# ChainSafe/co-zkvms

Measured on AMD Instinct MI355X. Metric: RISC-V cycles proved/sec (co-Jolt hot path: PST13 commit + dense GKR grand product + openings), higher is better.
Workload: dtype u32-limb BN254 Fr/Fq (254-bit Montgomery integers); 1 GPU; configs[1] restated (SURVEY 8d): 2^20-cycle trace per GPU, plain prover, 128 polys (64 Fr + 32 u16 + 16 u32 + 16 flags) PST13 batch commit, dense grand product 8 x 2^21 leaves, batch evaluate + opening reduction + PST13 open; log_n=20, polys=128, gp_batch=8, parallelism=single GPU, ranks_per_gpu=1

## Files before the change

co-zkvms_amd/csrc/capi.hip:

```cpp
#include "common.hpp"
#include "fq9.hip.hpp"
#include "prf.hip.hpp"

static __device__ __forceinline__ uint64_t splitmix_next(uint64_t& s) {
    s += 0x9E3779B97F4A7C15ull;
    uint64_t z = s;
    z = (z ^ (z >> 30)) * 0xBF58476D1CE4E5B9ull;
    z = (z ^ (z >> 27)) * 0x94D049BB133111EBull;
    return z ^ (z >> 31);
}

__global__ void k_fill_random_fr(fe* out, size_t n, uint64_t seed, int max_bits) {
    size_t i = (size_t)blockIdx.x * blockDim.x + threadIdx.x;
    if (i >= n) return;
    uint64_t s = seed + (uint64_t)i * 0xD1342543DE82EF95ull;
    fe v;
    for (;;) {
        uint64_t w0 = splitmix_next(s), w1 = splitmix_next(s), w2 = splitmix_next(s);
        uint64_t w3 = splitmix_next(s) & ((1ull << 62) - 1ull);
        v.l[0] = (uint32_t)w0; v.l[1] = (uint32_t)(w0 >> 32);
        v.l[2] = (uint32_t)w1; v.l[3] = (uint32_t)(w1 >> 32);
        v.l[4] = (uint32_t)w2; v.l[5] = (uint32_t)(w2 >> 32);
        v.l[6] = (uint32_t)w3; v.l[7] = (uint32_t)(w3 >> 32);
        if (!Fr::geq_mod(v)) break;
// ... 116 lines not shown
    {
        std::lock_guard<std::mutex> lk(g_ctx_mu);
        g_live_ctx.insert(ctx);
    }
    *out = ctx;
    return COZK_OK;
}

int cozk_ctx_destroy(cozk_ctx* ctx) {
    if (!ctx) return COZK_OK;
    {
        std::lock_guard<std::mutex> lk(g_ctx_mu);
        g_live_ctx.erase(ctx);
    }
    (void)hipSetDevice(ctx->device);
    (void)hipStreamSynchronize(ctx->stream);
    if (ctx->ring_comm) (void)cozk_ring_destroy(ctx);
    ctx->pool.destroy();
    for (auto& pr : ctx->prof_events) {
        (void)hipEventDestroy(pr.first);
        (void)hipEventDestroy(pr.second);
    }
    for (ProfSlot& sl : ctx->prof_slots) sl.reset();
    ctx->msm_ws.release();
    ctx->scratch.release();
    ctx->scratch2.release();
    if (ctx->pinned) (void)hipHostFree(ctx->pinned);
    if (ctx->round_flag) (void)hipHostFree(ctx->round_flag);
    if (ctx->finish_ticket) (void)hipFree(ctx->finish_ticket);
    if (ctx->mailbox) (void)hipHostFree(ctx->mailbox);
    if (ctx->stream2) {
        (void)hipStreamSynchronize(ctx->stream2);
        (void)hipStreamDestroy(ctx->stream2);
    }
    (void)hipStreamDestroy(ctx->stream);
    delete ctx;
    return COZK_OK;
}

int cozk_ctx_set_resident_rounds(cozk_ctx* ctx, int enable) {
    if (!ctx) return COZK_ERR_INVALID_ARG;
    ctx->resident_rounds = enable > 0 ? 1 : (enable == 0 ? 0 : -1);
    return COZK_OK;
}

const char* cozk_last_error(cozk_ctx* ctx) { return ctx ? ctx->last_error.c_str() : "null context"; }

int cozk_ctx_synchronize(cozk_ctx* ctx) {
    return cozk_guard(ctx, [&] { HIP_TRY(hipStreamSynchronize(ctx->stream)); });
}

int cozk_ctx_stream(cozk_ctx* ctx, void** out_stream) {
    if (!ctx || !out_stream) return COZK_ERR_INVALID_ARG;
    *out_stream = (void*)ctx->stream;
    return COZK_OK;
}

int cozk_vec_alloc(cozk_ctx* ctx, size_t n, int kind, cozk_vec** out) {
    return cozk_guard(ctx, [&] {
        COZK_REQUIRE(ctx && out && scalar_kind_bytes(kind), "vec_alloc: bad argument");
        size_t bytes = n * scalar_kind_bytes(kind);
        void* d = ctx_dev_alloc(ctx, bytes);
        *out = new cozk_vec{ctx, n, kind, d, bytes, true};
    });
}

// ... 233 lines not shown
```

co-zkvms_amd/csrc/common.hpp:

```cpp
#pragma once
#ifdef COZK_COUNT_COPIES
#include <hip/hip_runtime.h>
#include <map>
#include <string>
#include <cstdio>
#include <mutex>
struct CozkCopyCounter {
    std::map<std::string, unsigned long> m;
    std::mutex mu;
    ~CozkCopyCounter() {
        for (auto& kv : m) fprintf(stderr, "[copies] %8lu  %s\n", kv.second, kv.first.c_str());
    }
};
inline CozkCopyCounter& cozk_copy_counter() { static CozkCopyCounter c; return c; }
inline void cozk_count_copy(const char* what, const char* f, int l) {
    auto& c = cozk_copy_counter();
    std::lock_guard<std::mutex> g(c.mu);
    const char* b = f;
    for (const char* p = f; *p; p++) if (*p == '/') b = p + 1;
    c.m[std::string(what) + " " + b + ":" + std::to_string(l)]++;
}
#define hipMemcpyAsync(...) (cozk_count_copy("memcpy", __FILE__, __LINE__), hipMemcpyAsync(__VA_ARGS__))
#define hipStreamSynchronize(...) (cozk_count_copy("sync", __FILE__, __LINE__), hipStreamSynchronize(__VA_ARGS__))
#define hipMemsetAsync(...) (cozk_count_copy("memset", __FILE__, __LINE__), hipMemsetAsync(__VA_ARGS__))
// ... 41 lines not shown
    void reserve(size_t bytes) {
        if (bytes <= cap) return;
        if (p) HIP_TRY(hipFree(p));
        p = nullptr;
        cap = 0;
        if (hipMalloc(&p, bytes) != hipSuccess) {
            (void)hipGetLastError();
            p = nullptr;
            trim_current_pool();
            HIP_TRY(hipMalloc(&p, bytes));
        }
        cap = bytes;
    }
    void release() {
        if (p) (void)hipFree(p);
        p = nullptr;
        cap = 0;
    }
    template <class T>
    T* as() { return reinterpret_cast<T*>(p); }
};

struct MsmSortWs {
    DevBuf hist, off0, refs, offA, ptrs;
    hipEvent_t done = nullptr, consumed = nullptr;
    void release() {
        for (DevBuf* b : {&hist, &off0, &refs, &offA, &ptrs}) b->release();
        for (hipEvent_t* e : {&done, &consumed}) {
            if (*e) (void)hipEventDestroy(*e);
            *e = nullptr;
        }
    }
};
struct MsmWorkspace {
    MsmSortWs sort[2];
    DevBuf offB, offC, heavy, partA, partB, bsum, chunk, grp, out, ptrs, exc, blk, perm, offP, form, corr;
    hipEvent_t fork = nullptr;
    void* pin = nullptr;
    size_t pin_cap = 0;
    void release() {
        for (MsmSortWs& s : sort) s.release();
        for (DevBuf* b : {&offB, &offC, &heavy, &partA, &partB, &bsum, &chunk, &grp, &out, &ptrs, &exc, &blk, &perm, &offP, &form, &corr}) b->release();
        if (pin) (void)hipHostFree(pin);
        pin = nullptr;
        pin_cap = 0;
        if (fork) (void)hipEventDestroy(fork);
        fork = nullptr;
    }
};

struct DevPool {
    std::unordered_map<size_t, std::vector<void*>> parked;
    std::unordered_map<void*, size_t> live;
    size_t parked_bytes = 0;
    size_t live_bytes = 0, peak_bytes = 0;
    void count(size_t c) {
        live_bytes += c;
        if (live_bytes > peak_bytes) peak_bytes = live_bytes;
    }
    static size_t size_class(size_t bytes) {
        if (bytes <= 256) return 256;
        size_t top = (size_t)1 << (63 - __builtin_clzll((unsigned long long)bytes));
        size_t q = top >> 2;
        return (bytes + q - 1) / q * q;
    }
    void trim() {
        for (auto& kv : parked)
            for (void* p : kv.second) (void)hipFree(p);
        parked.clear();
        parked_bytes = 0;
    }
    void* alloc(size_t bytes) {
        size_t c = size_class(bytes);
        auto it = parked.find(c);
        if (it != parked.end() && !it->second.empty()) {
            void* p = it->second.back();
            it->second.pop_back();
            parked_bytes -= c;
            live[p] = c;
            count(c);
// ... 23 lines not shown
        trim();
        for (auto& kv : live) (void)hipFree(kv.first);
        live.clear();
    }
};

enum {
    COZK_PROF_EVAL_CHI = 0,
    COZK_PROF_LINCOMB,
    COZK_PROF_BIND_CUBIC,
    COZK_PROF_MSM_SCATTER,
    COZK_PROF_LAYER_OUTPUT,
    COZK_PROF_SLOTS
};
struct ProfSlot {
    std::vector<std::pair<hipEvent_t, hipEvent_t>> events;
    double ms = 0.0;
    uint64_t launches = 0, alg_bytes = 0;
    void reset() {
        for (auto& pr : events) {
            (void)hipEventDestroy(pr.first);
            (void)hipEventDestroy(pr.second);
        }
        events.clear();
        ms = 0.0;
        launches = alg_bytes = 0;
    }
};

struct cozk_ctx {
    int device = 0;
    hipStream_t stream = nullptr;
    hipStream_t stream2 = nullptr;
    DevPool pool;
    std::string last_error;
    MsmWorkspace msm_ws;
    DevBuf scratch;
    DevBuf scratch2;
    void* pinned = nullptr;
    size_t pinned_cap = 0;
    int resident_rounds = -1;
    void* mailbox = nullptr;
    uint32_t* round_flag = nullptr;
    uint32_t round_seq = 0;
    uint32_t armed_seq = 0;
    unsigned* finish_ticket = nullptr;
    bool prof_enabled = false;
    std::vector<std::pair<hipEvent_t, hipEvent_t>> prof_events;
    double prof_ms = 0.0;
    uint64_t prof_launches = 0;
    uint64_t prof_units = 0;
    uint64_t prof_alg_bytes = 0;
    ProfSlot prof_slots[COZK_PROF_SLOTS];
    void* ring_comm = nullptr;
    int ring_rank = 0, ring_n = 0;
    uint64_t ring_bytes = 0;
    cozk_sparse_stats sparse_stats{};
};

struct ProfScope {
    cozk_ctx* ctx;
    hipStream_t st;
    int slot;
    hipEvent_t e0 = nullptr, e1 = nullptr;
    ProfScope(cozk_ctx* c, int slot_, uint64_t alg_bytes, hipStream_t stream = nullptr) : ctx(c), st(stream ? stream : c->stream), slot(slot_) {
        if (!ctx->prof_enabled) return;
// ... 123 lines not shown
```

co-zkvms_amd/csrc/msm.hip:

```cpp
#include "common.hpp"
#include "fq9.hip.hpp"
#include <cstring>

static constexpr uint32_t NB = 1u << 15;
static constexpr int CH = 16;
static constexpr int TPB = 256;

template <int KIND>
struct ScalarKind;
template <>
struct ScalarKind<COZK_SCALAR_FR> {
    static constexpr int NWIN = 16;
    static __device__ __forceinline__ bool load(const void* p, size_t i, uint32_t w[8]) {
        fe s = Fr::from_mont(fe_load(reinterpret_cast<const fe*>(p) + i));
#pragma unroll
        for (int k = 0; k < 8; k++) w[k] = s.l[k];
        return false;
    }
};
template <>
struct ScalarKind<COZK_SCALAR_U8> {
    static constexpr int NWIN = 1;
    static __device__ __forceinline__ bool load(const void* p, size_t i, uint32_t w[8]) {
        w[0] = reinterpret_cast<const uint8_t*>(p)[i];
// ... 749 lines not shown
        if (m > pl.bound) pl.bound = m;
    }
    COZK_REQUIRE(pl.M < (1ull << 32), "msm: batch too large (reference count exceeds 32 bits)");
    uint32_t L0 = (uint32_t)(pl.M >> 18);
    if (L0 < 8) L0 = 8;
    if (L0 > 127) L0 = 127;
    pl.L0 = L0;
    pl.maxseg0 = pl.M / L0 + pl.nb;
    uint64_t per = 0;
    for (size_t p = 0; p < P; p++) {
        uint64_t m = ((uint64_t)ns[p] * (pl.pre ? kind_nwin(kinds[p]) : 1) + NB - 1) / NB;
        if (m > per) per = m;
    }
    uint64_t segs = (per * 5 + 4 * L0 - 1) / (4 * L0) + 1;
    pl.fold_levels = 1;
    while ((segs = (segs + 7) / 8) > 1) pl.fold_levels++;
    return pl;
}

static void msm_scan(hipStream_t st, uint32_t* bsums, uint32_t nb, bool from_offsets, const uint32_t* in, uint32_t L, uint32_t* off, uint32_t* cursor,
                     const uint32_t* perm = nullptr) {
    const uint32_t nscan_blocks = (nb + SCAN_PER_BLOCK - 1) / SCAN_PER_BLOCK;
    if (from_offsets) {
        k_scan_sums<true><<<nscan_blocks, 256, 0, st>>>(in, nb, L, bsums, perm);
        k_scan_top<<<1, 1024, 0, st>>>(bsums, nscan_blocks, off + nb);
        k_scan_final<true><<<nscan_blocks, 256, 0, st>>>(in, nb, L, bsums, off, cursor, perm);
    } else {
        k_scan_sums<false><<<nscan_blocks, 256, 0, st>>>(in, nb, L, bsums, nullptr);
        k_scan_top<<<1, 1024, 0, st>>>(bsums, nscan_blocks, off + nb);
        k_scan_final<false><<<nscan_blocks, 256, 0, st>>>(in, nb, L, bsums, off, cursor, nullptr);
    }
}

static void msm_sort(cozk_ctx* ctx, hipStream_t st, MsmSortWs& sw, const MsmSetPlan& pl, const cozk_bases* bases, const size_t* offsets,
                     const size_t* ns, const void* const* scalars, const int* kinds) {
    const uint32_t nb = pl.nb, G = pl.G;
    const size_t P = pl.P;
    sw.hist.reserve((size_t)(nb + 3) * 4);
    sw.off0.reserve((size_t)(nb + 1) * 4);
    sw.offA.reserve((size_t)(nb + 1) * 4);
    sw.refs.reserve((size_t)pl.M * 4);
    uint32_t* hist = sw.hist.as<uint32_t>();
    uint32_t* off0 = sw.off0.as<uint32_t>();
    uint32_t* refs = sw.refs.as<uint32_t>();
    const uint32_t nscan_blocks = (nb + SCAN_PER_BLOCK - 1) / SCAN_PER_BLOCK;
    sw.ptrs.reserve((size_t)nscan_blocks * 4 + P * sizeof(MsmPolyDesc) + 64);
    uint32_t* bsums = sw.ptrs.as<uint32_t>();
    MsmPolyDesc* d_descs = reinterpret_cast<MsmPolyDesc*>(((uintptr_t)(bsums + nscan_blocks) + 15) & ~(uintptr_t)15);
    HIP_TRY(hipMemsetAsync(hist, 0, (size_t)(nb + 3) * 4, st));
    uint32_t* d_stats = hist + nb + 1;
    auto fullest_bucket = [&] { k_max_u32<<<std::min<uint32_t>(cdiv(nb, 256), 1024u), 256, 0, st>>>(hist, nb, d_stats); };
    auto read_back_stats = [&] {
        k_msm_set_total<<<1, 1, 0, st>>>(off0 + nb, d_stats);
        HIP_TRY(hipMemcpyAsync(&pl.pin->fullest, d_stats, 8, hipMemcpyDeviceToHost, st));
    };
    if (pl.pre) {
        MsmPolyDesc* h_descs = pl.pin->descs;
        COZK_REQUIRE(P <= 64, "msm: too many polynomials in one launch set");
        uint32_t nd = 0;
        struct KindRun { int kind; uint32_t first, count; size_t max_n; uint32_t wgs; };
        std::vector<KindRun> runs;
        size_t max_n = 0;
        for (int kind = 0; kind <= COZK_SCALAR_I64; kind++) {
            KindRun r{kind, nd, 0, 0, 0};
            for (size_t p = 0; p < P; p++)
                if (kinds[p] == kind && ns[p]) {
                    h_descs[nd++] = MsmPolyDesc{scalars[p], (uint32_t)ns[p], (uint32_t)offsets[p], (uint32_t)p, 0};
                    if (ns[p] > r.max_n) r.max_n = ns[p];
                }
            r.count = nd - r.first;
            if (r.max_n > max_n) max_n = r.max_n;
            if (r.count) runs.push_back(r);
        }
        HIP_TRY(hipMemcpyAsync(d_descs, h_descs, nd * sizeof(MsmPolyDesc), hipMemcpyHostToDevice, st));
        static const int ltpb_env = getenv("COZK_MSM_LTPB") ? atoi(getenv("COZK_MSM_LTPB")) : 0;
        static const int wgs_env = getenv("COZK_MSM_WGS") ? atoi(getenv("COZK_MSM_WGS")) : 0;
        const int ltpb = ltpb_env ? ltpb_env : (pl.wide ? MSM_WIDE_LTPB : 256);
        const uint32_t wgs_max = (uint32_t)(wgs_env ? wgs_env : (pl.wide ? MSM_WIDE_WGS : 64));
        COZK_REQUIRE(ltpb >= 64 && ltpb <= LTPB && ltpb % 64 == 0, "COZK_MSM_LTPB out of range");
// ... 22 lines not shown
        fullest_bucket();
        msm_scan(st, bsums, nb, false, hist, 1, off0, hist);
        read_back_stats();
        for (auto& r : runs) {
            dim3 grid(r.wgs, r.count);
            uint64_t alg = 0;
            for (uint32_t q = 0; q < r.count; q++) {
                const MsmPolyDesc& d = h_descs[r.first + q];
                const uint64_t sb = scalar_kind_bytes(r.kind);
                alg += (uint64_t)d.n * (sb + 4ull * ((sb * 8 + 15) / 16));
            }
            ProfScope prof(ctx, COZK_PROF_MSM_SCATTER, alg, st);
            KIND_DISPATCH(r.kind, (k_msm_scatter_lds<K><<<grid, ltpb, 0, st>>>(d_descs + r.first, hist, refs, (uint32_t)bases->n, pl.form)));
        }
    } else {
        for (size_t p = 0; p < P; p++) {
            uint32_t* h = hist + (size_t)p * G * NB;
            if (ns[p]) KIND_DISPATCH(kinds[p], (k_msm_hist<K><<<cdiv(ns[p], TPB), TPB, 0, st>>>(scalars[p], ns[p], h, 1)));
        }
        fullest_bucket();
        msm_scan(st, bsums, nb, false, hist, 1, off0, hist);
        read_back_stats();
        for (size_t p = 0; p < P; p++) {
            uint32_t* cur = hist + (size_t)p * G * NB;
            if (ns[p])
                KIND_DISPATCH(kinds[p], (k_msm_scatter<K><<<cdiv(ns[p], TPB), TPB, 0, st>>>(scalars[p], ns[p], cur, refs, 1, (uint32_t)bases->n,
                                                                                         (uint32_t)offsets[p])));
        }
    }
    msm_scan(st, bsums, nb, true, off0, pl.L0, sw.offA.as<uint32_t>(), nullptr);
    HIP_TRY(hipGetLastError());
}

static void msm_accumulate(cozk_ctx* ctx, MsmSortWs& sw, const MsmSetPlan& pl, const cozk_bases* bases, const size_t* ns, const int* kinds,
                           g1_xyzz* dense_out) {
    MsmWorkspace& ws = ctx->msm_ws;
    hipStream_t st = ctx->stream;
    const uint32_t nb = pl.nb, L0 = pl.L0;
    const uint32_t L1 = 8;
    const uint64_t maxseg0 = pl.maxseg0;
    const uint64_t maxpart = maxseg0 > 2ull * nb ? maxseg0 : 2ull * nb;
    ws.partA.reserve((size_t)maxpart * sizeof(g1_xyzz));
    ws.partB.reserve((size_t)maxpart * sizeof(g1_xyzz));
    ws.offB.reserve((size_t)(nb + 1) * 4);
    ws.offC.reserve((size_t)(nb + 1) * 4);
    ws.heavy.reserve((size_t)(nb + 1) * 4);
    ws.ptrs.reserve((size_t)((nb + SCAN_PER_BLOCK - 1) / SCAN_PER_BLOCK) * 4 + 64);
    uint32_t* refs = sw.refs.as<uint32_t>();
    uint32_t* off0 = sw.off0.as<uint32_t>();
    uint32_t* offA = sw.offA.as<uint32_t>();
    hipEvent_t e0 = nullptr, e1 = nullptr;
    if (ctx->prof_enabled) {
        HIP_TRY(hipEventCreate(&e0));
        HIP_TRY(hipEventCreate(&e1));
        HIP_TRY(hipEventRecord(e0, st));
    }
    ws.blk.reserve((size_t)(cdiv(maxpart, TPB) + 2) * 4);
    uint32_t* blk = ws.blk.as<uint32_t>();
    if (pl.pre) {
        ws.exc.reserve((size_t)(maxseg0 + 2) * 4);
        uint32_t* exc = ws.exc.as<uint32_t>();
        HIP_TRY(hipMemsetAsync(exc, 0, 4, st));
        ws.perm.reserve((size_t)nb * 4);
        ws.offP.reserve((size_t)(nb + 1) * 4 + SEGKEYS * 4);
        uint32_t* perm = ws.perm.as<uint32_t>();
        uint32_t* offP = ws.offP.as<uint32_t>();
        uint32_t* bins = offP + nb + 1;
        HIP_TRY(hipMemsetAsync(bins, 0, SEGKEYS * 4, st));
        k_seg_hist<<<cdiv(nb, 1024), 1024, 0, st>>>(off0, offA, nb, bins);
        k_seg_bins<<<1, 1, 0, st>>>(bins);
        k_seg_perm<<<cdiv(nb, 1024), 1024, 0, st>>>(off0, offA, nb, bins, perm);
        msm_scan(st, ws.ptrs.as<uint32_t>(), nb, true, offA, 1, offP, nullptr, perm);
        const uint32_t nblk0 = cdiv(maxseg0, TPB);
        k_block_buckets<<<cdiv(nblk0 + 1, 256), 256, 0, st>>>(offP, nb, nblk0, blk);
        if (bases->has_inf)
            k_msm_accum0_f9<true><<<nblk0, TPB, 0, st>>>(bases->table, refs, off0, offA, nb, ws.partA.as<g1_xyzz>(), exc, blk, offP, perm);
        else
            k_msm_accum0_f9<false, true><<<nblk0, TPB, 0, st>>>(bases->table, refs, off0, offA, nb, ws.partA.as<g1_xyzz>(), exc, blk, offP, perm);
        k_msm_accum0_fix<<<256, TPB, 0, st>>>(bases->table, refs, off0, offA, nb, ws.partA.as<g1_xyzz>(), exc, offP, perm);
    } else {
        k_msm_accum0<<<cdiv(maxseg0, TPB), TPB, 0, st>>>(bases->table, refs, off0, offA, nb, L0, ws.partA.as<g1_xyzz>());
    }
    if (ctx->prof_enabled) {
        HIP_TRY(hipEventRecord(e1, st));
        ctx->prof_events.push_back({e0, e1});
        ctx->prof_launches += 1;
        for (size_t p = 0; p < pl.P; p++) ctx->prof_alg_bytes += (uint64_t)ns[p] * (64 + scalar_kind_bytes(kinds[p]));
    }
    uint32_t* heavy = ws.heavy.as<uint32_t>();
    HIP_TRY(hipMemsetAsync(heavy, 0, 4, st));
    uint64_t maxseg = maxseg0;
    g1_xyzz* cur_items = ws.partA.as<g1_xyzz>();
    g1_xyzz* nxt_items = ws.partB.as<g1_xyzz>();
    uint32_t* cur_off = offA;
    uint32_t* nxt_off = ws.offB.as<uint32_t>();
    uint32_t* spare_off = ws.offC.as<uint32_t>();
    for (uint32_t level = 0; level < pl.fold_levels; level++) {
        uint64_t nseg = maxseg / L1 + nb;
        msm_scan(st, ws.ptrs.as<uint32_t>(), nb, true, cur_off, L1, nxt_off, nullptr);
        const uint32_t nblkN = cdiv(nseg, TPB);
        k_block_buckets<<<cdiv(nblkN + 1, 256), 256, 0, st>>>(nxt_off, nb, nblkN, blk);
        k_msm_accumN<<<nblkN, TPB, 0, st>>>(cur_items, cur_off, nxt_off, nb, L1, nxt_items, blk);
        std::swap(cur_items, nxt_items);
        uint32_t* done = cur_off;
        cur_off = nxt_off;
        nxt_off = (done == offA) ? spare_off : done;
        maxseg = nseg;
    }
    k_msm_gather_buckets<<<cdiv(nb, TPB), TPB, 0, st>>>(cur_items, cur_off, nb, dense_out, heavy);
    k_msm_fold_heavy<<<HEAVY_GRID, TPB, 0, st>>>(cur_items, cur_off, heavy, dense_out);
    HIP_TRY(hipGetLastError());
}

static void affine_to_abi(const g1_affine& a, uint64_t xy[8], int* inf) {
    bool is_inf = G1::is_inf(a);
    for (int i = 0; i < 4; i++) {
        xy[i] = (uint64_t)a.x.l[2 * i] | ((uint64_t)a.x.l[2 * i + 1] << 32);
        xy[4 + i] = (uint64_t)a.y.l[2 * i] | ((uint64_t)a.y.l[2 * i + 1] << 32);
    }
    if (inf) *inf = is_inf ? 1 : 0;
}
static g1_affine abi_to_affine(const uint64_t xy[8], int inf) {
    g1_affine a;
    for (int i = 0; i < 4; i++) {
        a.x.l[2 * i] = (uint32_t)xy[i];
        a.x.l[2 * i + 1] = (uint32_t)(xy[i] >> 32);
        a.y.l[2 * i] = (uint32_t)xy[4 + i];
        a.y.l[2 * i + 1] = (uint32_t)(xy[4 + i] >> 32);
    }
    if (inf) {
        a.x = Fq::zero();
        a.y = Fq::zero();
    }
    return a;
}

void msm_batch(cozk_ctx* ctx, const cozk_bases* bases, const size_t* offsets, const size_t* ns, const void* const* scalars,
               const int* kinds, size_t k, uint64_t* out_xy, int* out_inf);

enum { MSM_FORM_AUTO = 0, MSM_FORM_PLAIN = 1, MSM_FORM_OFFSET = 2 };
static int msm_digit_form_mode() {
    const char* e = getenv("COZK_MSM_DIGIT_FORM");
    if (!e || !*e || !strcmp(e, "auto")) return MSM_FORM_AUTO;
    if (!strcmp(e, "plain")) return MSM_FORM_PLAIN;
    if (!strcmp(e, "offset")) return MSM_FORM_OFFSET;
    throw CozkError(COZK_ERR_INVALID_ARG, "COZK_MSM_DIGIT_FORM must be auto, plain or offset");
}

struct MsmSchedule {
    bool shape_rule = true;
    int wg_digits_log2 = MSM_WG_DIGITS_LOG2;
};
static MsmSchedule msm_schedule_env() {
    MsmSchedule s;
    if (const char* e = getenv("COZK_MSM_SHAPE_RULE")) s.shape_rule = atoi(e) != 0;
    if (const char* e = getenv("COZK_MSM_WG_DIGITS_LOG2")) {
        s.wg_digits_log2 = atoi(e);
        COZK_REQUIRE(s.wg_digits_log2 == 0 || (s.wg_digits_log2 >= 10 && s.wg_digits_log2 <= 24), "COZK_MSM_WG_DIGITS_LOG2 must be 0 or 10..24");
    }
    return s;
}

static constexpr size_t MSM_SLICE_SUMS = 32;
static cozk_bases::SliceSum msm_slice_sum(cozk_ctx* ctx, const cozk_bases* bases, size_t off, size_t n) {
    cozk_bases* b = const_cast<cozk_bases*>(bases);
    {
        std::lock_guard<std::mutex> lk(b->sums_mu);
        for (const auto& e : b->sums)
            if (e.off == off && e.n == n) return e;
    }
    void* ones = ctx_dev_alloc(ctx, n);
    uint64_t xy[8];
    int inf = 0;
    try {
        HIP_TRY(hipMemsetAsync(ones, 1, n, ctx->stream));
        const void* p = ones;
        int kind = COZK_SCALAR_U8;
        msm_batch(ctx, bases, &off, &n, &p, &kind, 1, xy, &inf);
    } catch (...) {
        ctx_dev_free(ctx, ones);
        throw;
    }
    ctx_dev_free(ctx, ones);
    const g1_affine S = abi_to_affine(xy, inf);
    cozk_bases::SliceSum e;
    e.off = off;
    e.n = n;
    const uint64_t c[3] = {0x8000ull, 0x80008000ull, 0x8000800080008000ull};
    for (int j = 0; j < 3; j++) {
        g1_xyzz acc = G1::identity();
        for (int bit = 63; bit >= 0; bit--) {
            acc = G1::dbl(acc);
            if ((c[j] >> bit) & 1ull) acc = G1::add_mixed(acc, S);
        }
        e.cS[j] = G1::to_affine(acc);
    }
    std::lock_guard<std::mutex> lk(b->sums_mu);
    for (const auto& have : b->sums)
        if (have.off == off && have.n == n) return have;
    if (b->sums.size() >= MSM_SLICE_SUMS) b->sums.erase(b->sums.begin());
    b->sums.push_back(e);
    return e;
}

void msm_batch(cozk_ctx* ctx, const cozk_bases* bases, const size_t* offsets, const size_t* ns, const void* const* scalars,
               const int* kinds, size_t k, uint64_t* out_xy, int* out_inf) {
    MsmWorkspace& ws = ctx->msm_ws;
    hipStream_t st = ctx->stream;
    const uint32_t G = bases->nwin == 16 ? 1u : 16u;
    const size_t maxP = bases->nwin == 16 ? 64 : 4;
    const size_t tail_cap = 256 / G;
    const int form_mode = msm_digit_form_mode();
    const MsmSchedule sched = msm_schedule_env();
    std::vector<uint8_t> elig(k, 0);
    std::vector<g1_affine> corr_h;
    bool any_elig = false;
    if (G == 1 && form_mode != MSM_FORM_PLAIN) {
        for (size_t p = 0; p < k; p++) {
            const int slot = kind_offset_slot(kinds[p]);
            if (slot < 0 || ns[p] == 0) continue;
            COZK_REQUIRE(offsets[p] + ns[p] <= bases->n, "msm: base slice out of range");
            if (!any_elig) corr_h.assign(k, g1_affine{Fq::zero(), Fq::zero()});
            any_elig = true;
            elig[p] = 1;
            if (p > 0 && elig[p - 1] && kinds[p - 1] == kinds[p] && offsets[p - 1] == offsets[p] && ns[p - 1] == ns[p]) corr_h[p] = corr_h[p - 1];
            else corr_h[p] = msm_slice_sum(ctx, bases, offsets[p], ns[p]).cS[slot];
        }
    }
    ws.out.reserve(k * sizeof(g1_affine));
    g1_affine* d_out = ws.out.as<g1_affine>();
    const size_t pin_need = k * (sizeof(MsmSetPin) + sizeof(g1_affine));
    if (pin_need > ws.pin_cap) {
        if (ws.pin) (void)hipHostFree(ws.pin);
        ws.pin = nullptr;
        ws.pin_cap = 0;
        HIP_TRY(hipHostMalloc(&ws.pin, pin_need, hipHostMallocDefault));
        ws.pin_cap = pin_need;
    }
    MsmSetPin* pins = reinterpret_cast<MsmSetPin*>(ws.pin);
// ... 32 lines not shown
                if (set_refs_cap < (1ull << 28)) set_refs_cap = 1ull << 28;
                if (set_refs_cap > (1ull << 30)) set_refs_cap = 1ull << 30;
            }
        }
        {
            size_t s = 0;
            while (s < kt) {
                size_t P = 0;
                uint64_t M = 0;
                while (s + P < kt && P < maxP) {
                    uint64_t m = (uint64_t)ns[t0 + s + P] * kind_nwin(kinds[t0 + s + P]);
                    if (P > 0 && M + m > set_refs_cap) break;
                    M += m;
                    P++;
                }
                sets.push_back({s, P});
                s += P;
            }
        }
        if (sets.size() > 2) {
            size_t best = 0;
            uint64_t best_m = ~0ull;
            for (size_t i = 0; i < sets.size(); i++) {
                uint64_t m = 0;
                for (size_t p = 0; p < sets[i].P; p++) m += (uint64_t)ns[t0 + sets[i].s + p] * kind_nwin(kinds[t0 + sets[i].s + p]);
                if (m < best_m) {
                    best_m = m;
                    best = i;
                }
            }
            std::rotate(sets.begin(), sets.begin() + best, sets.begin() + best + 1);
        }
        static const bool pipeline = getenv("COZK_MSM_SERIAL") == nullptr;
        hipStream_t side = st;
        if (pipeline && sets.size() > 1) {
            if (!ctx->stream2) {
                static const bool prio = getenv("COZK_MSM_NO_PRIORITY") == nullptr;
                int lo = 0, hi = 0;
                HIP_TRY(hipDeviceGetStreamPriorityRange(&lo, &hi));
                if (prio) HIP_TRY(hipStreamCreateWithPriority(&ctx->stream2, hipStreamNonBlocking, hi));
                else HIP_TRY(hipStreamCreateWithFlags(&ctx->stream2, hipStreamNonBlocking));
            }
            side = ctx->stream2;
        }
        for (int b = 0; b < 2; b++) {
            if (!ws.sort[b].done) HIP_TRY(hipEventCreateWithFlags(&ws.sort[b].done, hipEventDisableTiming));
            if (!ws.sort[b].consumed) HIP_TRY(hipEventCreateWithFlags(&ws.sort[b].consumed, hipEventDisableTiming));
        }
        if (side != st) {
            if (!ws.fork) HIP_TRY(hipEventCreateWithFlags(&ws.fork, hipEventDisableTiming));
            HIP_TRY(hipEventRecord(ws.fork, st));
            HIP_TRY(hipStreamWaitEvent(side, ws.fork, 0));
        }
        std::vector<MsmSetPlan> plans(sets.size());
        auto launch_sort = [&](size_t i) {
            const SetRange& r = sets[i];
            plans[i] = msm_plan(bases, offsets + t0 + r.s, ns + t0 + r.s, kinds + t0 + r.s, r.P);
            if (plans[i].M == 0) return;
            MsmSetPlan& pl = plans[i];
            pl.pin = pins + pins_used++;
            pl.pin->fullest = 0;
            pl.pin->total = 0;
            pin_bound.push_back(pl.bound);
            pl.form = any_elig ? d_form + t0 + r.s : nullptr;
            pl.counts = any_elig ? d_counts + 2 * (t0 + r.s) : nullptr;
            for (size_t p = 0; p < r.P; p++)
                if (elig[t0 + r.s + p]) pl.elig |= 1ull << p;
            pl.force_offset = form_mode == MSM_FORM_OFFSET;
            const uint64_t pred_refs = i > 0 && side != st ? plans[i - 1].M : 0;
            pl.wide = sched.shape_rule ? msm_sort_wide(pred_refs, pl.M) : (i == 0 && t0 == 0) || side == st;
            pl.wg_digits_log2 = sched.wg_digits_log2;
            pl.index = (uint32_t)i;
            MsmSortWs& sw = ws.sort[i & 1];
            if (i >= 2 && side != st) HIP_TRY(hipStreamWaitEvent(side, sw.consumed, 0));
            msm_sort(ctx, side, sw, plans[i], bases, offsets + t0 + r.s, ns + t0 + r.s, scalars + t0 + r.s, kinds + t0 + r.s);
            if (side != st) HIP_TRY(hipEventRecord(sw.done, side));
        };
        if (!sets.empty()) launch_sort(0);
        for (size_t i = 0; i < sets.size(); i++) {
            if (side != st && i + 1 < sets.size()) launch_sort(i + 1);
            const SetRange& r = sets[i];
            g1_xyzz* out_i = dense + (size_t)r.s * G * NB;
            if (plans[i].M != 0) {
                MsmSortWs& sw = ws.sort[i & 1];
                if (side != st) HIP_TRY(hipStreamWaitEvent(st, sw.done, 0));
                msm_accumulate(ctx, sw, plans[i], bases, ns + t0 + r.s, kinds + t0 + r.s, out_i);
                if (side != st) HIP_TRY(hipEventRecord(sw.consumed, st));
            } else {
                HIP_TRY(hipMemsetAsync(out_i, 0, (size_t)plans[i].nb * sizeof(g1_xyzz), st));
            }
            if (side == st && i + 1 < sets.size()) launch_sort(i + 1);
        }
        k_msm_reduce_chunks<<<cdiv((uint64_t)ngroups * (NB / CH), TPB), TPB, 0, st>>>(dense, ngroups, ws.chunk.as<g1_xyzz>());
        k_msm_reduce_groups<<<ngroups, TPB, 0, st>>>(ws.chunk.as<g1_xyzz>(), ws.grp.as<g1_xyzz>());
        k_msm_finalize<<<cdiv(kt, 64), 64, 0, st>>>(ws.grp.as<g1_xyzz>(), G, (uint32_t)kt, d_out + t0, d_form ? d_form + t0 : nullptr,
                                                   d_corr ? d_corr + t0 : nullptr);
        HIP_TRY(hipGetLastError());
    }
    g1_affine* h = reinterpret_cast<g1_affine*>(ctx_pinned(ctx, k * sizeof(g1_affine)));
    HIP_TRY(hipMemcpyAsync(h, d_out, k * sizeof(g1_affine), hipMemcpyDeviceToHost, st));
    HIP_TRY(hipStreamSynchronize(st));
    for (size_t i = 0; i < pins_used; i++) {
        COZK_REQUIRE(pins[i].fullest <= pin_bound[i], "msm: histogram larger than the reference count");
        if (ctx->prof_enabled) ctx->prof_units += pins[i].total;
    }
    for (size_t i = 0; i < k; i++) affine_to_abi(h[i], out_xy + 8 * i, out_inf ? out_inf + i : nullptr);
}

extern "C" {

int cozk_bases_upload(cozk_ctx* ctx, const uint64_t* xy, const uint8_t* infinity, size_t n, int precompute,
                      cozk_bases** out) {
    return cozk_guard(ctx, [&] {
        COZK_REQUIRE(ctx && xy && out && n > 0, "bases_upload: bad argument");
        cozk_bases* b = new cozk_bases{ctx, n, precompute ? 16 : 1, nullptr};
        try {
            HIP_TRY(hipMalloc((void**)&b->table, (size_t)b->nwin * n * sizeof(g1_affine)));
            std::vector<g1_affine> h(n);
            for (size_t i = 0; i < n; i++) h[i] = abi_to_affine(xy + 8 * i, infinity ? infinity[i] : 0);
            HIP_TRY(hipMemcpyAsync(b->table, h.data(), n * sizeof(g1_affine), hipMemcpyHostToDevice, ctx->stream));
            HIP_TRY(hipStreamSynchronize(ctx->stream));
            build_window_table(ctx, b);
            HIP_TRY(hipStreamSynchronize(ctx->stream));
        } catch (...) {
            if (b->table) (void)hipFree(b->table);
            delete b;
            throw;
// ... 216 lines not shown
```

Before: 9.248 million cycles/s.

## Run MSM bucket folds on a third stream with per-set reduction tails

Splits MSM accumulation into a gather phase on the main stream and a fold phase on a new third stream. Fold workspaces are double-buffered and all buffers are reserved up front, draining the streams if a buffer must grow. The per-set reduce kernels are also issued right after each set's fold instead of once at the end. The aim is to overlap the fold and reduce tail of one set with the sort and gather of the next set. The cost is an extra device-to-device copy of offA per set, more events and cross-stream waits, and higher memory use from duplicated fold buffers.

```diff
diff --git a/co-zkvms_amd/csrc/capi.hip b/co-zkvms_amd/csrc/capi.hip
--- a/co-zkvms_amd/csrc/capi.hip
+++ b/co-zkvms_amd/csrc/capi.hip
@@ -172,6 +172,10 @@
     if (ctx->stream2) {
         (void)hipStreamSynchronize(ctx->stream2);
         (void)hipStreamDestroy(ctx->stream2);
+    }
+    if (ctx->stream3) {
+        (void)hipStreamSynchronize(ctx->stream3);
+        (void)hipStreamDestroy(ctx->stream3);
     }
     (void)hipStreamDestroy(ctx->stream);
     delete ctx;
diff --git a/co-zkvms_amd/csrc/common.hpp b/co-zkvms_amd/csrc/common.hpp
--- a/co-zkvms_amd/csrc/common.hpp
+++ b/co-zkvms_amd/csrc/common.hpp
@@ -97,20 +97,35 @@
         }
     }
 };
+struct MsmFoldWs {
+    DevBuf partA, partB, offB, offC, heavy, blk, ptrs;
+    hipEvent_t gathered = nullptr, folded = nullptr;
+    void release() {
+        for (DevBuf* b : {&partA, &partB, &offB, &offC, &heavy, &blk, &ptrs}) b->release();
+        for (hipEvent_t* e : {&gathered, &folded}) {
+            if (*e) (void)hipEventDestroy(*e);
+            *e = nullptr;
+        }
+    }
+};
 struct MsmWorkspace {
     MsmSortWs sort[2];
-    DevBuf offB, offC, heavy, partA, partB, bsum, chunk, grp, out, ptrs, exc, blk, perm, offP, form, corr;
-    hipEvent_t fork = nullptr;
+    MsmFoldWs fold[2];
+    DevBuf bsum, chunk, grp, out, ptrs, exc, blk, perm, offP, form, corr;
+    hipEvent_t fork = nullptr, join = nullptr;
     void* pin = nullptr;
     size_t pin_cap = 0;
     void release() {
         for (MsmSortWs& s : sort) s.release();
-        for (DevBuf* b : {&offB, &offC, &heavy, &partA, &partB, &bsum, &chunk, &grp, &out, &ptrs, &exc, &blk, &perm, &offP, &form, &corr}) b->release();
+        for (MsmFoldWs& f : fold) f.release();
+        for (DevBuf* b : {&bsum, &chunk, &grp, &out, &ptrs, &exc, &blk, &perm, &offP, &form, &corr}) b->release();
         if (pin) (void)hipHostFree(pin);
         pin = nullptr;
         pin_cap = 0;
-        if (fork) (void)hipEventDestroy(fork);
-        fork = nullptr;
+        for (hipEvent_t* e : {&fork, &join}) {
+            if (*e) (void)hipEventDestroy(*e);
+            *e = nullptr;
+        }
     }
 };
 
@@ -200,6 +215,7 @@
     int device = 0;
     hipStream_t stream = nullptr;
     hipStream_t stream2 = nullptr;
+    hipStream_t stream3 = nullptr;
     DevPool pool;
     std::string last_error;
     MsmWorkspace msm_ws;
diff --git a/co-zkvms_amd/csrc/msm.hip b/co-zkvms_amd/csrc/msm.hip
--- a/co-zkvms_amd/csrc/msm.hip
+++ b/co-zkvms_amd/csrc/msm.hip
@@ -805,19 +805,70 @@
     }
 }
 
+static void msm_drain(cozk_ctx* ctx) {
+    for (hipStream_t s : {ctx->stream, ctx->stream2, ctx->stream3})
+        if (s) (void)hipStreamSynchronize(s);
+}
+
+struct MsmReserve {
+    cozk_ctx* ctx;
+    bool in_flight;
+    void operator()(DevBuf& b, size_t bytes) {
+        if (bytes <= b.cap) return;
+        if (in_flight) msm_drain(ctx);
+        in_flight = false;
+        b.reserve(bytes);
+    }
+};
+static uint64_t msm_maxpart(const MsmSetPlan& pl) { return pl.maxseg0 > 2ull * pl.nb ? pl.maxseg0 : 2ull * pl.nb; }
+static void msm_reserve_prep(MsmReserve& grow, DevBuf& exc, DevBuf& perm, DevBuf& offP, DevBuf& blk, const MsmSetPlan& pl) {
+    grow(exc, (size_t)(pl.maxseg0 + 2) * 4);
+    grow(perm, (size_t)pl.nb * 4);
+    grow(offP, (size_t)(pl.nb + 1) * 4 + SEGKEYS * 4);
+    grow(blk, (size_t)(cdiv(pl.maxseg0, TPB) + 2) * 4);
+}
+static void msm_reserve_sort(MsmReserve& grow, MsmSortWs& sw, const MsmSetPlan& pl) {
+    const uint32_t nb = pl.nb;
+    grow(sw.hist, (size_t)(nb + 3) * 4);
+    grow(sw.off0, (size_t)(nb + 1) * 4);
+    grow(sw.offA, (size_t)(nb + 1) * 4);
+    grow(sw.refs, (size_t)pl.M * 4);
+    grow(sw.ptrs, (size_t)cdiv(nb, SCAN_PER_BLOCK) * 4 + pl.P * sizeof(MsmPolyDesc) + 64);
+}
+static void msm_reserve_fold(MsmReserve& grow, MsmFoldWs& fw, const MsmSetPlan& pl) {
+    const uint32_t nb = pl.nb;
+    const uint64_t maxpart = msm_maxpart(pl);
+    grow(fw.partA, (size_t)maxpart * sizeof(g1_xyzz));
+    grow(fw.partB, (size_t)maxpart * sizeof(g1_xyzz));
+    grow(fw.offB, (size_t)(nb + 1) * 4);
+    grow(fw.offC, (size_t)(nb + 1) * 4);
+    grow(fw.heavy, (size_t)(nb + 1) * 4);
+    grow(fw.blk, (size_t)(cdiv(maxpart, TPB) + 2) * 4);
+    grow(fw.ptrs, (size_t)cdiv(nb, SCAN_PER_BLOCK) * 4 + 64);
+}
+
+static void msm_prepare(hipStream_t st, const MsmSetPlan& pl, const uint32_t* off0, const uint32_t* offA, uint32_t* bsums, uint32_t* exc,
+                        uint32_t* perm, uint32_t* offP, uint32_t* blk) {
+    const uint32_t nb = pl.nb;
+    HIP_TRY(hipMemsetAsync(exc, 0, 4, st));
+    uint32_t* bins = offP + nb + 1;
+    HIP_TRY(hipMemsetAsync(bins, 0, SEGKEYS * 4, st));
+    k_seg_hist<<<cdiv(nb, 1024), 1024, 0, st>>>(off0, offA, nb, bins);
+    k_seg_bins<<<1, 1, 0, st>>>(bins);
+    k_seg_perm<<<cdiv(nb, 1024), 1024, 0, st>>>(off0, offA, nb, bins, perm);
+    msm_scan(st, bsums, nb, true, offA, 1, offP, nullptr, perm);
+    const uint32_t nblk0 = cdiv(pl.maxseg0, TPB);
+    k_block_buckets<<<cdiv(nblk0 + 1, 256), 256, 0, st>>>(offP, nb, nblk0, blk);
+}
+
 static void msm_sort(cozk_ctx* ctx, hipStream_t st, MsmSortWs& sw, const MsmSetPlan& pl, const cozk_bases* bases, const size_t* offsets,
                      const size_t* ns, const void* const* scalars, const int* kinds) {
     const uint32_t nb = pl.nb, G = pl.G;
     const size_t P = pl.P;
-    sw.hist.reserve((size_t)(nb + 3) * 4);
-    sw.off0.reserve((size_t)(nb + 1) * 4);
-    sw.offA.reserve((size_t)(nb + 1) * 4);
-    sw.refs.reserve((size_t)pl.M * 4);
     uint32_t* hist = sw.hist.as<uint32_t>();
     uint32_t* off0 = sw.off0.as<uint32_t>();
     uint32_t* refs = sw.refs.as<uint32_t>();
     const uint32_t nscan_blocks = (nb + SCAN_PER_BLOCK - 1) / SCAN_PER_BLOCK;
-    sw.ptrs.reserve((size_t)nscan_blocks * 4 + P * sizeof(MsmPolyDesc) + 64);
     uint32_t* bsums = sw.ptrs.as<uint32_t>();
     MsmPolyDesc* d_descs = reinterpret_cast<MsmPolyDesc*>(((uintptr_t)(bsums + nscan_blocks) + 15) & ~(uintptr_t)15);
     HIP_TRY(hipMemsetAsync(hist, 0, (size_t)(nb + 3) * 4, st));
@@ -906,75 +957,73 @@
     HIP_TRY(hipGetLastError());
 }
 
-static void msm_accumulate(cozk_ctx* ctx, MsmSortWs& sw, const MsmSetPlan& pl, const cozk_bases* bases, const size_t* ns, const int* kinds,
-                           g1_xyzz* dense_out) {
+static void msm_gather(cozk_ctx* ctx, MsmSortWs& sw, MsmFoldWs& fw, const MsmSetPlan& pl, const cozk_bases* bases, const size_t* ns,
+                       const int* kinds) {
     MsmWorkspace& ws = ctx->msm_ws;
     hipStream_t st = ctx->stream;
     const uint32_t nb = pl.nb, L0 = pl.L0;
-    const uint32_t L1 = 8;
     const uint64_t maxseg0 = pl.maxseg0;
-    const uint64_t maxpart = maxseg0 > 2ull * nb ? maxseg0 : 2ull * nb;
-    ws.partA.reserve((size_t)maxpart * sizeof(g1_xyzz));
-    ws.partB.reserve((size_t)maxpart * sizeof(g1_xyzz));
-    ws.offB.reserve((size_t)(nb + 1) * 4);
-    ws.offC.reserve((size_t)(nb + 1) * 4);
-    ws.heavy.reserve((size_t)(nb + 1) * 4);
-    ws.ptrs.reserve((size_t)((nb + SCAN_PER_BLOCK - 1) / SCAN_PER_BLOCK) * 4 + 64);
     uint32_t* refs = sw.refs.as<uint32_t>();
     uint32_t* off0 = sw.off0.as<uint32_t>();
     uint32_t* offA = sw.offA.as<uint32_t>();
+    g1_xyzz* part = fw.partA.as<g1_xyzz>();
     hipEvent_t e0 = nullptr, e1 = nullptr;
-    if (ctx->prof_enabled) {
+    auto prof_begin = [&] {
+        if (!ctx->prof_enabled) return;
         HIP_TRY(hipEventCreate(&e0));
         HIP_TRY(hipEventCreate(&e1));
         HIP_TRY(hipEventRecord(e0, st));
-    }
-    ws.blk.reserve((size_t)(cdiv(maxpart, TPB) + 2) * 4);
-    uint32_t* blk = ws.blk.as<uint32_t>();
-    if (pl.pre) {
-        ws.exc.reserve((size_t)(maxseg0 + 2) * 4);
-        uint32_t* exc = ws.exc.as<uint32_t>();
-        HIP_TRY(hipMemsetAsync(exc, 0, 4, st));
-        ws.perm.reserve((size_t)nb * 4);
-        ws.offP.reserve((size_t)(nb + 1) * 4 + SEGKEYS * 4);
-        uint32_t* perm = ws.perm.as<uint32_t>();
-        uint32_t* offP = ws.offP.as<uint32_t>();
-        uint32_t* bins = offP + nb + 1;
-        HIP_TRY(hipMemsetAsync(bins, 0, SEGKEYS * 4, st));
-        k_seg_hist<<<cdiv(nb, 1024), 1024, 0, st>>>(off0, offA, nb, bins);
-        k_seg_bins<<<1, 1, 0, st>>>(bins);
-        k_seg_perm<<<cdiv(nb, 1024), 1024, 0, st>>>(off0, offA, nb, bins, perm);
-        msm_scan(st, ws.ptrs.as<uint32_t>(), nb, true, offA, 1, offP, nullptr, perm);
-        const uint32_t nblk0 = cdiv(maxseg0, TPB);
-        k_block_buckets<<<cdiv(nblk0 + 1, 256), 256, 0, st>>>(offP, nb, nblk0, blk);
-        if (bases->has_inf)
-            k_msm_accum0_f9<true><<<nblk0, TPB, 0, st>>>(bases->table, refs, off0, offA, nb, ws.partA.as<g1_xyzz>(), exc, blk, offP, perm);
-        else
-            k_msm_accum0_f9<false, true><<<nblk0, TPB, 0, st>>>(bases->table, refs, off0, offA, nb, ws.partA.as<g1_xyzz>(), exc, blk, offP, perm);
-        k_msm_accum0_fix<<<256, TPB, 0, st>>>(bases->table, refs, off0, offA, nb, ws.partA.as<g1_xyzz>(), exc, offP, perm);
-    } else {
-        k_msm_accum0<<<cdiv(maxseg0, TPB), TPB, 0, st>>>(bases->table, refs, off0, offA, nb, L0, ws.partA.as<g1_xyzz>());
-    }
-    if (ctx->prof_enabled) {
+    };
+    auto prof_end = [&] {
+        if (!ctx->prof_enabled) return;
         HIP_TRY(hipEventRecord(e1, st));
         ctx->prof_events.push_back({e0, e1});
         ctx->prof_launches += 1;
         for (size_t p = 0; p < pl.P; p++) ctx->prof_alg_bytes += (uint64_t)ns[p] * (64 + scalar_kind_bytes(kinds[p]));
-    }
-    uint32_t* heavy = ws.heavy.as<uint32_t>();
+    };
+    if (pl.pre) {
+        uint32_t* exc = ws.exc.as<uint32_t>();
+        uint32_t* perm = ws.perm.as<uint32_t>();
+        uint32_t* offP = ws.offP.as<uint32_t>();
+        uint32_t* blk = ws.blk.as<uint32_t>();
+        msm_prepare(st, pl, off0, offA, ws.ptrs.as<uint32_t>(), exc, perm, offP, blk);
+        const uint32_t nblk0 = cdiv(maxseg0, TPB);
+        prof_begin();
+        if (bases->has_inf)
+            k_msm_accum0_f9<true><<<nblk0, TPB, 0, st>>>(bases->table, refs, off0, offA, nb, part, exc, blk, offP, perm);
+        else
+            k_msm_accum0_f9<false, true><<<nblk0, TPB, 0, st>>>(bases->table, refs, off0, offA, nb, part, exc, blk, offP, perm);
+        prof_end();
+        k_msm_accum0_fix<<<256, TPB, 0, st>>>(bases->table, refs, off0, offA, nb, part, exc, offP, perm);
+    } else {
+        prof_begin();
+        k_msm_accum0<<<cdiv(maxseg0, TPB), TPB, 0, st>>>(bases->table, refs, off0, offA, nb, L0, part);
+        prof_end();
+    }
+    HIP_TRY(hipGetLastError());
+}
+
+static void msm_fold(hipStream_t st, MsmSortWs& sw, MsmFoldWs& fw, const MsmSetPlan& pl, g1_xyzz* dense_out, hipEvent_t consumed,
+                     bool own_offA) {
+    const uint32_t nb = pl.nb;
+    const uint32_t L1 = 8;
+    uint32_t* offA = sw.offA.as<uint32_t>();
+    uint32_t* blk = fw.blk.as<uint32_t>();
+    uint32_t* heavy = fw.heavy.as<uint32_t>();
     HIP_TRY(hipMemsetAsync(heavy, 0, 4, st));
-    uint64_t maxseg = maxseg0;
-    g1_xyzz* cur_items = ws.partA.as<g1_xyzz>();
-    g1_xyzz* nxt_items = ws.partB.as<g1_xyzz>();
-    uint32_t* cur_off = offA;
-    uint32_t* nxt_off = ws.offB.as<uint32_t>();
-    uint32_t* spare_off = ws.offC.as<uint32_t>();
+    uint64_t maxseg = pl.maxseg0;
+    g1_xyzz* cur_items = fw.partA.as<g1_xyzz>();
+    g1_xyzz* nxt_items = fw.partB.as<g1_xyzz>();
+    uint32_t* cur_off = own_offA ? fw.offC.as<uint32_t>() : offA;
+    uint32_t* nxt_off = fw.offB.as<uint32_t>();
+    uint32_t* spare_off = fw.offC.as<uint32_t>();
     for (uint32_t level = 0; level < pl.fold_levels; level++) {
         uint64_t nseg = maxseg / L1 + nb;
-        msm_scan(st, ws.ptrs.as<uint32_t>(), nb, true, cur_off, L1, nxt_off, nullptr);
+        msm_scan(st, fw.ptrs.as<uint32_t>(), nb, true, cur_off, L1, nxt_off, nullptr);
         const uint32_t nblkN = cdiv(nseg, TPB);
         k_block_buckets<<<cdiv(nblkN + 1, 256), 256, 0, st>>>(nxt_off, nb, nblkN, blk);
         k_msm_accumN<<<nblkN, TPB, 0, st>>>(cur_items, cur_off, nxt_off, nb, L1, nxt_items, blk);
+        if (level == 0 && consumed) HIP_TRY(hipEventRecord(consumed, st));
         std::swap(cur_items, nxt_items);
         uint32_t* done = cur_off;
         cur_off = nxt_off;
@@ -984,6 +1033,11 @@
     k_msm_gather_buckets<<<cdiv(nb, TPB), TPB, 0, st>>>(cur_items, cur_off, nb, dense_out, heavy);
     k_msm_fold_heavy<<<HEAVY_GRID, TPB, 0, st>>>(cur_items, cur_off, heavy, dense_out);
     HIP_TRY(hipGetLastError());
+}
+
+static void msm_reduce(hipStream_t st, const g1_xyzz* dense, uint32_t ngroups, g1_xyzz* chunk, g1_xyzz* grp) {
+    k_msm_reduce_chunks<<<cdiv((uint64_t)ngroups * (NB / CH), TPB), TPB, 0, st>>>(dense, ngroups, chunk);
+    k_msm_reduce_groups<<<ngroups, TPB, 0, st>>>(chunk, grp);
 }
 
 static void affine_to_abi(const g1_affine& a, uint64_t xy[8], int* inf) {
@@ -1024,9 +1078,18 @@
 struct MsmSchedule {
     bool shape_rule = true;
     int wg_digits_log2 = MSM_WG_DIGITS_LOG2;
+    bool fold_stream = true, tail_per_set = true;
 };
 static MsmSchedule msm_schedule_env() {
     MsmSchedule s;
+    if (const char* e = getenv("COZK_MSM_OVERLAP"); e && *e) {
+        s.fold_stream = s.tail_per_set = false;
+        if (strcmp(e, "0") != 0)
+            for (; *e; e++) {
+                COZK_REQUIRE(*e == 'b' || *e == 'c', "COZK_MSM_OVERLAP must be 0 or a combination of b and c");
+                (*e == 'b' ? s.fold_stream : s.tail_per_set) = true;
+            }
+    }
     if (const char* e = getenv("COZK_MSM_SHAPE_RULE")) s.shape_rule = atoi(e) != 0;
     if (const char* e = getenv("COZK_MSM_WG_DIGITS_LOG2")) {
         s.wg_digits_log2 = atoi(e);
@@ -1077,8 +1140,19 @@
     return e;
 }
 
+static void msm_batch_streams(cozk_ctx* ctx, const cozk_bases* bases, const size_t* offsets, const size_t* ns, const void* const* scalars,
+                              const int* kinds, size_t k, uint64_t* out_xy, int* out_inf);
 void msm_batch(cozk_ctx* ctx, const cozk_bases* bases, const size_t* offsets, const size_t* ns, const void* const* scalars,
                const int* kinds, size_t k, uint64_t* out_xy, int* out_inf) {
+    try {
+        msm_batch_streams(ctx, bases, offsets, ns, scalars, kinds, k, out_xy, out_inf);
+    } catch (...) {
+        msm_drain(ctx);
+        throw;
+    }
+}
+static void msm_batch_streams(cozk_ctx* ctx, const cozk_bases* bases, const size_t* offsets, const size_t* ns, const void* const* scalars,
+                              const int* kinds, size_t k, uint64_t* out_xy, int* out_inf) {
     MsmWorkspace& ws = ctx->msm_ws;
     hipStream_t st = ctx->stream;
     const uint32_t G = bases->nwin == 16 ? 1u : 16u;
@@ -1177,30 +1251,48 @@
             std::rotate(sets.begin(), sets.begin() + best, sets.begin() + best + 1);
         }
         static const bool pipeline = getenv("COZK_MSM_SERIAL") == nullptr;
-        hipStream_t side = st;
-        if (pipeline && sets.size() > 1) {
-            if (!ctx->stream2) {
+        hipStream_t side = st, folds = st;
+        auto side_stream = [&](hipStream_t* s) {
+            if (!*s) {
                 static const bool prio = getenv("COZK_MSM_NO_PRIORITY") == nullptr;
                 int lo = 0, hi = 0;
                 HIP_TRY(hipDeviceGetStreamPriorityRange(&lo, &hi));
-                if (prio) HIP_TRY(hipStreamCreateWithPriority(&ctx->stream2, hipStreamNonBlocking, hi));
-                else HIP_TRY(hipStreamCreateWithFlags(&ctx->stream2, hipStreamNonBlocking));
+                if (prio) HIP_TRY(hipStreamCreateWithPriority(s, hipStreamNonBlocking, hi));
+                else HIP_TRY(hipStreamCreateWithFlags(s, hipStreamNonBlocking));
             }
-            side = ctx->stream2;
-        }
-        for (int b = 0; b < 2; b++) {
-            if (!ws.sort[b].done) HIP_TRY(hipEventCreateWithFlags(&ws.sort[b].done, hipEventDisableTiming));
-            if (!ws.sort[b].consumed) HIP_TRY(hipEventCreateWithFlags(&ws.sort[b].consumed, hipEventDisableTiming));
+            return *s;
+        };
+        const bool piped = pipeline && sets.size() > 1;
+        if (piped) {
+            side = side_stream(&ctx->stream2);
+            if (sched.fold_stream) folds = side_stream(&ctx->stream3);
+        }
+        const bool tail_per_set = piped && sched.tail_per_set;
+        for (hipEvent_t* e : {&ws.sort[0].done, &ws.sort[0].consumed, &ws.sort[1].done, &ws.sort[1].consumed, &ws.fold[0].gathered,
+                              &ws.fold[0].folded, &ws.fold[1].gathered, &ws.fold[1].folded, &ws.fork, &ws.join})
+            if (!*e) HIP_TRY(hipEventCreateWithFlags(e, hipEventDisableTiming));
+        std::vector<MsmSetPlan> plans(sets.size());
+        {
+            MsmReserve grow{ctx, t0 != 0};
+            for (size_t i = 0; i < sets.size(); i++) {
+                const SetRange& r = sets[i];
+                MsmSetPlan& pl = plans[i] = msm_plan(bases, offsets + t0 + r.s, ns + t0 + r.s, kinds + t0 + r.s, r.P);
+                if (pl.M == 0) continue;
+                msm_reserve_sort(grow, ws.sort[i & 1], pl);
+                msm_reserve_fold(grow, ws.fold[folds != st ? i & 1 : 0], pl);
+                if (pl.pre) {
+                    msm_reserve_prep(grow, ws.exc, ws.perm, ws.offP, ws.blk, pl);
+                    grow(ws.ptrs, (size_t)cdiv(pl.nb, SCAN_PER_BLOCK) * 4 + 64);
+                }
+            }
         }
         if (side != st) {
-            if (!ws.fork) HIP_TRY(hipEventCreateWithFlags(&ws.fork, hipEventDisableTiming));
             HIP_TRY(hipEventRecord(ws.fork, st));
             HIP_TRY(hipStreamWaitEvent(side, ws.fork, 0));
-        }
-        std::vector<MsmSetPlan> plans(sets.size());
+            if (folds != st) HIP_TRY(hipStreamWaitEvent(folds, ws.fork, 0));
+        }
         auto launch_sort = [&](size_t i) {
             const SetRange& r = sets[i];
-            plans[i] = msm_plan(bases, offsets + t0 + r.s, ns + t0 + r.s, kinds + t0 + r.s, r.P);
             if (plans[i].M == 0) return;
             MsmSetPlan& pl = plans[i];
             pl.pin = pins + pins_used++;
@@ -1228,16 +1320,30 @@
             g1_xyzz* out_i = dense + (size_t)r.s * G * NB;
             if (plans[i].M != 0) {
                 MsmSortWs& sw = ws.sort[i & 1];
+                MsmFoldWs& fw = ws.fold[folds != st ? i & 1 : 0];
                 if (side != st) HIP_TRY(hipStreamWaitEvent(st, sw.done, 0));
-                msm_accumulate(ctx, sw, plans[i], bases, ns + t0 + r.s, kinds + t0 + r.s, out_i);
-                if (side != st) HIP_TRY(hipEventRecord(sw.consumed, st));
+                if (folds != st && i >= 2) HIP_TRY(hipStreamWaitEvent(st, fw.folded, 0));
+                msm_gather(ctx, sw, fw, plans[i], bases, ns + t0 + r.s, kinds + t0 + r.s);
+                if (folds != st) {
+                    HIP_TRY(hipMemcpyAsync(fw.offC.as<uint32_t>(), sw.offA.as<uint32_t>(), (size_t)(plans[i].nb + 1) * 4, hipMemcpyDeviceToDevice, st));
+                    HIP_TRY(hipEventRecord(sw.consumed, st));
+                    HIP_TRY(hipEventRecord(fw.gathered, st));
+                    HIP_TRY(hipStreamWaitEvent(folds, fw.gathered, 0));
+                }
+                msm_fold(folds, sw, fw, plans[i], out_i, side != st && folds == st ? sw.consumed : nullptr, folds != st);
+                if (folds != st) HIP_TRY(hipEventRecord(fw.folded, folds));
             } else {
-                HIP_TRY(hipMemsetAsync(out_i, 0, (size_t)plans[i].nb * sizeof(g1_xyzz), st));
+                HIP_TRY(hipMemsetAsync(out_i, 0, (size_t)plans[i].nb * sizeof(g1_xyzz), folds));
             }
+            if (tail_per_set)
+                msm_reduce(folds, out_i, (uint32_t)r.P * G, ws.chunk.as<g1_xyzz>() + (size_t)r.s * G * (NB / CH), ws.grp.as<g1_xyzz>() + (size_t)r.s * G);
             if (side == st && i + 1 < sets.size()) launch_sort(i + 1);
         }
-        k_msm_reduce_chunks<<<cdiv((uint64_t)ngroups * (NB / CH), TPB), TPB, 0, st>>>(dense, ngroups, ws.chunk.as<g1_xyzz>());
-        k_msm_reduce_groups<<<ngroups, TPB, 0, st>>>(ws.chunk.as<g1_xyzz>(), ws.grp.as<g1_xyzz>());
+        if (folds != st) {
+            HIP_TRY(hipEventRecord(ws.join, folds));
+            HIP_TRY(hipStreamWaitEvent(st, ws.join, 0));
+        }
+        if (!tail_per_set) msm_reduce(st, dense, ngroups, ws.chunk.as<g1_xyzz>(), ws.grp.as<g1_xyzz>());
         k_msm_finalize<<<cdiv(kt, 64), 64, 0, st>>>(ws.grp.as<g1_xyzz>(), G, (uint32_t)kt, d_out + t0, d_form ? d_form + t0 : nullptr,
                                                    d_corr ? d_corr + t0 : nullptr);
         HIP_TRY(hipGetLastError());
```

New measurement: 9.317 million cycles/s (median of 6 runs). No clear change (+0.8%).
